# nirvanesque/headCT_foundation

Measured on AMD Instinct MI355X. Metric: CT-volumes/sec MAE pretrain step (96^3, ViT-B/16^3, mask 0.75), higher is better.
Workload: dtype bf16; 1 GPU; BASELINE config #2: MAE ViT-B/16^3, 96^3x1ch, mask 0.75, full train step (fwd+bwd+clip+AdamW+LR); per_gpu_batch=256, global_batch=256, parallelism=dp1, init=reference init, seed 42

## Files before the change

### headct_foundation_amd/_lib.py

```python
from __future__ import annotations

import ctypes as C
import os
from typing import Optional

HERE = os.path.dirname(os.path.abspath(__file__))
LIB_PATH = os.path.join(HERE, "libheadct_hip.so")

HCT_F32, HCT_BF16, HCT_F16 = 0, 1, 2
NORM_LAYERNORM, NORM_RMSNORM = 0, 1
HCT_ACT_NONE, HCT_ACT_GELU, HCT_ACT_DGELU, HCT_ACT_TANH, HCT_ACT_GELU_D, HCT_ACT_MULAUX = 0, 1, 2, 3, 4, 5
ACT_NONE, ACT_GELU, ACT_DGELU = 0, 1, 2

c_void_p, c_int, c_float, c_size_t, c_int64 = C.c_void_p, C.c_int, C.c_float, C.c_size_t, C.c_int64


class GemmArgs(C.Structure):
    _fields_ = [
        ("M", c_int), ("N", c_int), ("K", c_int),
        ("A", c_void_p), ("a_dtype", c_int), ("lda", c_int64), ("transA", c_int),
        ("B", c_void_p), ("b_dtype", c_int), ("ldb", c_int64), ("transB", c_int),
        ("C", c_void_p), ("c_dtype", c_int), ("ldc", c_int64),
        ("bias", c_void_p), ("residual", c_void_p), ("ldr", c_int64),
        ("act", c_int),
        ("aux", c_void_p), ("aux_dtype", c_int), ("ldaux", c_int64),
        ("C2", c_void_p), ("c2_dtype", c_int), ("ldc2", c_int64),
        ("alpha", c_float), ("force_generic", c_int), ("colsum_out", c_void_p), ("workspace_armed", c_int),
    ]


class GemmPlanInfo(C.Structure):
    _fields_ = [("kernel", c_int), ("epilogue_mode", c_int), ("fuse_colsum", c_int), ("row_tiles_per_wave", c_int), ("tiles", c_int),
                ("grid", c_int), ("sk_tiles", c_int), ("sk_wgs", c_int), ("splits", c_int), ("r_chunk", c_int), ("colsum_bytes", c_size_t),
                ("stream_k_offset", c_size_t), ("slab_bytes", c_size_t), ("workspace_bytes", c_size_t)]


class ProfShape(C.Structure):
    _fields_ = [("M", c_int), ("N", c_int), ("K", c_int), ("mode", c_int), ("tiles", c_int), ("sk_tiles", c_int),
                ("launches", c_int64), ("total_ms", C.c_double), ("work", C.c_double), ("bytes", C.c_double)]


def prof_shapes(lib, kernel_class: int, cap: int = 256):
    buf = (ProfShape * cap)()
    n = lib.hct_prof_shapes(kernel_class, C.cast(buf, c_void_p), cap)
    if n < 0:
        raise HctError("hct_prof_shapes failed")
    return [buf[i] for i in range(min(n, cap))]


class MaeConfig(C.Structure):
    _fields_ = [
        ("input_size", c_int), ("patch_size", c_int), ("in_chans", c_int), ("mask_ratio", C.c_double),
        ("pos_embed", c_int),
        ("encoder_depth", c_int), ("encoder_embed_dim", c_int), ("encoder_mlp_dim", c_int), ("encoder_num_heads", c_int),
        ("decoder_depth", c_int), ("decoder_embed_dim", c_int), ("decoder_mlp_dim", c_int), ("decoder_num_heads", c_int),
        ("norm_pix_loss", c_int), ("use_bias", c_int),
        ("encoder_only", c_int), ("num_register_tokens", c_int), ("final_norm_eps", c_float),
        ("lora_rank", c_int),
        ("norm_kind", c_int),
        ("dropout_rate", c_float),
    ]


class ParamInfo(C.Structure):
    _fields_ = [
        ("name", C.c_char * 96), ("ndim", c_int), ("shape", c_int64 * 5), ("offset", c_int64), ("numel", c_int64),
        ("requires_grad", c_int), ("is_matrix", c_int), ("bf16_t_offset", c_int64),
    ]


_PROTOS = {
    "hct_last_error_string": (C.c_char_p, []),
    "hct_version": (c_int, []),
    "hct_has_mfma_kernels": (c_int, []),
    "hct_gemm_workspace_bytes": (c_size_t, [C.POINTER(GemmArgs)]),
    "hct_gemm_nt_flags_offset": (c_size_t, [c_size_t]),
    "hct_gemm_describe": (c_int, [C.POINTER(GemmArgs), c_int, c_size_t, C.POINTER(GemmPlanInfo)]),
    "hct_gemm_stream_k_items": (c_int, [c_int, c_int, c_int, c_int, C.POINTER(C.c_uint32), C.POINTER(C.c_uint32)]),
    "hct_set_cu_reserve": (None, [c_int]),
    "hct_gemm": (c_int, [C.POINTER(GemmArgs), c_void_p, c_size_t, c_void_p]),
    "hct_mask_rank": (c_int, [c_void_p, c_int, c_int, c_int, c_void_p, c_void_p, c_void_p, c_void_p]),
    "hct_patch_gather": (c_int, [c_void_p, c_int, c_void_p, c_int, c_int, c_int, c_int, c_int, c_int, c_void_p, c_int, c_void_p]),
    "hct_encoder_assemble_fwd": (c_int, [c_void_p, c_int, c_void_p, c_void_p, c_void_p, c_int, c_int, c_int, c_int, c_void_p, c_void_p]),
    "hct_encoder_assemble_bwd": (c_int, [c_void_p, c_void_p, c_int, c_int, c_int, c_int, c_void_p, c_int, c_void_p, c_void_p, c_void_p, c_size_t, c_void_p]),
    "hct_assemble_bwd_workspace_bytes": (c_size_t, [c_int]),
    "hct_layernorm_fwd": (c_int, [c_void_p, c_void_p, c_void_p, c_int, c_int, c_float, c_void_p, c_int, c_void_p, c_void_p, c_void_p]),
    "hct_layernorm_bwd_workspace_bytes": (c_size_t, [c_int, c_int]),
# ... 228 lines not shown
```

### headct_foundation_amd/csrc/gemm.hip

```cpp
#include "common.h"
#include "gemm_plan.h"
#include "prof.h"

#include <cstdlib>
#include <cstring>
#include <vector>

namespace hct {

struct Epilogue {
  const float* bias;
  const float* residual;
  int64_t ldr;
  int act;
  void* aux; int aux_dtype; int64_t ldaux;
  void* C; int c_dtype; int64_t ldc;
  void* C2; int c2_dtype; int64_t ldc2;
  float alpha;
  float* colsum_partial;
  int aux_deriv;
};

__device__ __forceinline__ void store4(void* base, int dtype, int64_t off, f32x4 v) {
  if (dtype == HCT_BF16) Vec4<bf16>::store((bf16*)base + off, v);
// ... 640 lines not shown
            for (int q = 0; q < 4; ++q) {
              x0[q] *= dgelu_fast((float)t[q]);
              x1[q] *= dgelu_fast((float)t[4 + q]);
            }
          }
          if (MODE == EPI_DGELU_CS) {
            cs[h][0] += ok ? x0 : f32x4{0, 0, 0, 0};
            cs[h][1] += ok ? x1 : f32x4{0, 0, 0, 0};
          }
        }
        __builtin_amdgcn_raw_buffer_store_b128(pack(x0, x1), tb.c, vc, sc, kBf16OutPolicy);
        HCT_STORE_GUARD();
      } else {
        const f32x4 v = *reinterpret_cast<const f32x4*>(patch + pr * 256 + ((cc ^ pr) << 4));
        f32x4 x = v * e.alpha + bias[h].lo;
        if (MODE == EPI_RES_F32) x += __builtin_bit_cast(f32x4, ld[s][it]);
        __builtin_amdgcn_raw_buffer_store_b128(__builtin_bit_cast(u32x4, x), tb.c, ok ? (lane_c + h * 64) * 4u : OOB, (row0 + prow) * ldc * 4, STORE_POLICY);
        HCT_STORE_GUARD();
      }
    }
  }
}


__device__ __forceinline__ i32x4 make_srd(const void* base, uint32_t num_records) {
  const uint64_t pa = (uint64_t)base;
  return i32x4{(int)__builtin_amdgcn_readfirstlane((uint32_t)pa), (int)(__builtin_amdgcn_readfirstlane((uint32_t)(pa >> 32)) & 0xFFFF),
               (int)__builtin_amdgcn_readfirstlane(num_records), 0x00020000};
}

__device__ __forceinline__ void dma16s(i32x4 rsrc, uint32_t lds_base, uint32_t voff, uint32_t soff) {
  asm volatile("s_mov_b32 m0, %0\n\ts_nop 0\n\tbuffer_load_dwordx4 %1, %2, %3 offen lds" ::"s"(lds_base), "v"(voff), "s"(rsrc), "s"(soff)
               : "memory", "m0");
}
__device__ __forceinline__ void dma16(i32x4 rsrc, uint32_t lds_base, uint32_t voff) {
  asm volatile("s_mov_b32 m0, %0\n\ts_nop 0\n\tbuffer_load_dwordx4 %1, %2, 0 offen lds" ::"s"(lds_base), "v"(voff), "s"(rsrc) : "memory", "m0");
}

#ifdef HCT_STAMPS
__device__ uint32_t* g_stamp_ptr = nullptr;
__device__ uint32_t g_stamp_words = 0;
#define HCT_STAMP(k)                                                                                   \
  do {                                                                                                 \
    unsigned long long t_;                                                                             \
    __builtin_amdgcn_sched_barrier(0);                                                                 \
    asm volatile("s_memrealtime %0\n\ts_waitcnt lgkmcnt(0)" : "=s"(t_)::"memory");                     \
    __builtin_amdgcn_sched_barrier(0);                                                                 \
    stamps = lane == ((tile_i * 4 + (k)) & 63) ? (uint32_t)t_ : stamps;                                \
  } while (0)
#else
#define HCT_STAMP(k)
#endif

constexpr int kSkErrWord = 512;

__device__ __forceinline__ unsigned sk_pub(unsigned seq_arg) { return ((seq_arg >> 31) ? seq_arg + 1u : seq_arg) & 0x0FFFFFFFu; }

__device__ __forceinline__ uint32_t xcc_id() {
  uint32_t v;
  asm volatile("s_getreg_b32 %0, hwreg(HW_REG_XCC_ID)" : "=s"(v));
  return v & 15;
}

template <int MODE, bool SK = false, int MT = 4>
__global__ void __launch_bounds__(512, 2) gemm_bf16_nt256_kernel(int M, int N, int K, const bf16* __restrict__ A, int64_t lda,
                                                                 const bf16* __restrict__ B, int64_t ldb, Epilogue e, int ntiles, int sk_tiles, int sk_wgs, unsigned char* __restrict__ sk_ws, unsigned sk_seq) {
  __shared__ __attribute__((aligned(16))) unsigned char smem[163840];
  static_assert(MT == 4 || (MT == 3 && !SK && (MODE == EPI_PLAIN_BF16 || MODE == EPI_RES_F32)), "192-row tiles: whole tiles, plain / +residual epilogues");
  const int lane = threadIdx.x & 63, wave = __builtin_amdgcn_readfirstlane(threadIdx.x >> 6);
  const int ntn = (N + 255) >> 8;
  float* const colsum_out = e.colsum_partial;

  constexpr int NP = 2;
  uint32_t voa[NP], vob[NP];
#pragma unroll
  for (int i = 0; i < NP; ++i) {
    const int row = ((wave & 7) * NP + i) * 16 + (lane >> 2);
    const int src_chunk = (lane & 3) ^ swz64(row);
    voa[i] = (uint32_t)(row * lda * 2 + src_chunk * 16);
    vob[i] = (uint32_t)(row * ldb * 2 + src_chunk * 16);
  }
  const int wm = wave >> 1, wn = wave & 1;
  const int frow = lane & 15, fchk = lane >> 4;
  const int foff = frow * 64 + ((fchk ^ swz64(frow)) << 4);
  const int nk = K >> 5;

  i32x4 ra, rb;
  const uint32_t lds0 = (uint32_t)(size_t)((__attribute__((address_space(3))) unsigned char*)smem);
  int m0 = 0, n0 = 0;
  auto set_tile_id = [&](int id, int s0) {
    const int tm = id / ntn, tn = id - tm * ntn;
    m0 = tm * (64 * MT);
    n0 = tn << 8;
    const bf16* Ab = A + (int64_t)m0 * lda + s0 * 32;
    const bf16* Bb = B + (int64_t)n0 * ldb + s0 * 32;
    ra = make_srd(Ab, clamp_records(((int64_t)(M - m0 - 1) * lda + K - s0 * 32) * 2));
    rb = make_srd(Bb, clamp_records(((int64_t)(N - n0 - 1) * ldb + K - s0 * 32) * 2));
  };
  auto dp_id = [&](int vb) {
    const int nwg = ntiles - sk_tiles;
    const int xcd = vb & 7, q = nwg >> 3, r = nwg & 7;
    return sk_tiles + (xcd < r ? xcd * (q + 1) : r * (q + 1) + (xcd - r) * q) + (vb >> 3);
  };
  auto stage_pair = [&](int t) {
    const uint32_t b0 = lds0 + (t % 5) * 32768, b1 = lds0 + ((t + 1) % 5) * 32768;
    const uint32_t kb = (uint32_t)t * 64;
#pragma unroll
    for (int i = 0; i < NP; ++i) {
      const int c = wave * NP + i;
      if (MT == 4 || c < 4 * MT) {
        dma16s(ra, b0 + c * 1024, voa[i], kb);
        dma16s(ra, b1 + c * 1024, voa[i], kb + 64);
      }
      dma16s(rb, b0 + 16384 + c * 1024, vob[i], kb);
      dma16s(rb, b1 + 16384 + c * 1024, vob[i], kb + 64);
    }
  };
  f32x4 acc[MT][8];
  bf16x8 b_lo[4], b_hi[4], a0[MT], a1[MT];
// ... 2 lines not shown
#pragma unroll
    for (int i = 0; i < MT; ++i) af[i] = *reinterpret_cast<const bf16x8*>(sa + i * 1024);
  };
  auto rd_b = [&](int t, int half, bf16x8* bq) {
    const unsigned char* sb = smem + (t % 5) * 32768 + 16384 + wn * (128 * 64) + half * 4096 + foff;
#pragma unroll
    for (int j = 0; j < 4; ++j) bq[j] = *reinterpret_cast<const bf16x8*>(sb + j * 1024);
  };
  auto mma = [&](int half, const bf16x8* af, const bf16x8* bq) {
#pragma unroll
    for (int i = 0; i < MT; ++i)
#pragma unroll
      for (int j = 0; j < 4; ++j)
        acc[i][half * 4 + j] = __builtin_amdgcn_mfma_f32_16x16x32_bf16(bq[j], af[i], acc[i][half * 4 + j], 0, 0, 0);
  };
  auto land_all = [&]() {
    asm volatile("s_waitcnt vmcnt(0)" ::: "memory");
    __builtin_amdgcn_s_barrier();
  };
  auto land_top = [&]() {
    if (MT == 3 && wave >= 6) asm volatile("s_waitcnt vmcnt(4)" ::: "memory");
    else asm volatile("s_waitcnt vmcnt(8)" ::: "memory");
    __builtin_amdgcn_s_barrier();
  };
#ifdef HCT_STAMPS
  uint32_t stamps = 0;
  int tile_i = 0;
#endif
  const int P = nk >> 1;
  uint32_t it_first = 0, it_owner = 0;
  if (SK) stream_k_items(blockIdx.x, sk_tiles, sk_wgs, P, it_first, it_owner);
  int vb = blockIdx.x;
  uint32_t cit = 0;
  auto take_item = [&](uint32_t it) {
    set_tile_id((int)(it & 255), (int)((it >> 8) & 1023) * 2);
    cit = it;
  };
  auto next_item = [&]() -> bool {
    if (SK && it_owner) {
      take_item(it_owner);
      it_owner = 0;
      return true;
    }
    if (vb < ntiles - sk_tiles) {
      set_tile_id(dp_id(vb), 0);
      cit = (uint32_t)P << 18;
      vb += gridDim.x;
      return true;
    }
    return false;
  };
  if (SK && it_first) take_item(it_first);
  else if (!next_item()) return;
  stage_pair(0);
  while (true) {
    HCT_STAMP(0);
    const int cm0 = m0, cn0 = n0;
    const uint32_t item = cit;
    const int cns = SK ? (int)((item >> 18) & 1023) * 2 : nk;
#pragma unroll
    for (int i = 0; i < MT; ++i)
#pragma unroll
      for (int j = 0; j < 8; ++j) acc[i][j] = f32x4{0, 0, 0, 0};
    __builtin_amdgcn_s_barrier();
    stage_pair(2);
    land_top();
    HCT_STAMP(1);
    rd_a(0, a0);
    rd_b(0, 0, b_lo);
    int t = 0;
    for (; t + 5 < cns; t += 2) {
      rd_b(t, 1, b_hi);
      mma(0, a0, b_lo);
      rd_a(t + 1, a1);
      rd_b(t + 1, 0, b_lo);
      mma(1, a0, b_hi);
      rd_b(t + 1, 1, b_hi);
      mma(0, a1, b_lo);
      land_all();
      stage_pair(t + 4);
      rd_a(t + 2, a0);
      rd_b(t + 2, 0, b_lo);
      mma(1, a1, b_hi);
    }
    rd_b(t, 1, b_hi);
    mma(0, a0, b_lo);
    rd_a(t + 1, a1);
    rd_b(t + 1, 0, b_lo);
    mma(1, a0, b_hi);
    rd_b(t + 1, 1, b_hi);
    mma(0, a1, b_lo);
    land_all();
    rd_a(t + 2, a0);
    rd_b(t + 2, 0, b_lo);
    mma(1, a1, b_hi);
    rd_b(t + 2, 1, b_hi);
    mma(0, a0, b_lo);
    rd_a(t + 3, a1);
    rd_b(t + 3, 0, b_lo);
    mma(1, a0, b_hi);
    TileBias bv = {f32x4{0, 0, 0, 0}, f32x4{0, 0, 0, 0}};
    TileBias bh[2] = {bv, bv};
    if (MODE != EPI_GENERIC) tile_bias_halves<MODE>(e, cn0, wn * 128, lane, N, bh);
    rd_b(t + 3, 1, b_hi);
    mma(0, a1, b_lo);
    mma(1, a1, b_hi);
// ... 676 lines not shown
__global__ void __launch_bounds__(256) gemm_fold_kernel(const float* __restrict__ slab, int splits, int M, int N, Epilogue e) {
  const int64_t total4 = (int64_t)M * N / 4;
  for (int64_t i = (int64_t)blockIdx.x * blockDim.x + threadIdx.x; i < total4; i += (int64_t)gridDim.x * blockDim.x) {
    const int64_t idx = i * 4;
    f32x4 s = Vec4<float>::load_nt(slab + idx);
    for (int z = 1; z < splits; ++z) s += Vec4<float>::load_nt(slab + (int64_t)z * M * N + idx);
    const int m = (int)(idx / N), n = (int)(idx - (int64_t)m * N);
    epilogue4(e, m, n, s);
  }
}

static int g_cu_reserve = 0;
static GemmTuning g_tuning;

static int num_cus_total() {
  static int n = 0;
  if (n == 0) {
    int dev = 0;
    hipDeviceProp_t prop;
    if (hipGetDevice(&dev) == hipSuccess && hipGetDeviceProperties(&prop, dev) == hipSuccess) n = prop.multiProcessorCount;
    if (n <= 0) n = 256;
  }
  return n;
}

static int num_cus() { return std::max(8, num_cus_total() - g_cu_reserve); }

static Epilogue make_epilogue(const hct_gemm_args* a) {
  Epilogue e;
  e.bias = a->bias; e.residual = a->residual; e.ldr = a->ldr;
  e.aux_deriv = a->act == HCT_ACT_GELU_D || a->act == HCT_ACT_MULAUX;
  e.act = a->act == HCT_ACT_GELU_D ? HCT_ACT_GELU : a->act == HCT_ACT_MULAUX ? HCT_ACT_DGELU : a->act;
  e.aux = a->aux; e.aux_dtype = a->aux_dtype; e.ldaux = a->ldaux;
  e.C = a->C; e.c_dtype = a->c_dtype; e.ldc = a->ldc;
  e.C2 = a->C2; e.c2_dtype = a->c2_dtype; e.ldc2 = a->ldc2;
  e.alpha = a->alpha;
  e.colsum_partial = nullptr;
  return e;
}

static unsigned next_sk_seq(unsigned& seq) {
  unsigned v = (++seq) & 0x0FFFFFFFu;
  if (v == 0) v = (++seq) & 0x0FFFFFFFu;
  return g_tuning.sk_drop ? v | 0x80000000u : v;
}

static int launch_nt256(const hct_gemm_args* a, const GemmPlan& p, Epilogue e, void* workspace, hipStream_t s) {
  if (p.fuse_colsum) e.colsum_partial = (float*)workspace;
  const dim3 grid(p.grid);
  const bf16 *A = (const bf16*)a->A, *B = (const bf16*)a->B;
  if (p.row_tiles_per_wave == 3) {
    if (p.epilogue_mode == EPI_PLAIN_BF16)
      hipLaunchKernelGGL((gemm_bf16_nt256_kernel<EPI_PLAIN_BF16, false, 3>), grid, dim3(512), 0, s, a->M, a->N, a->K, A, a->lda, B, a->ldb, e,
                         p.tiles, 0, 0, (unsigned char*)nullptr, 0u);
    else
      hipLaunchKernelGGL((gemm_bf16_nt256_kernel<EPI_RES_F32, false, 3>), grid, dim3(512), 0, s, a->M, a->N, a->K, A, a->lda, B, a->ldb, e,
                         p.tiles, 0, 0, (unsigned char*)nullptr, 0u);
    HCT_CHECK_LAUNCH("hct_gemm(nt256, 192-row tiles)");
    return 0;
  }
  unsigned char* sk_ws = nullptr;
  unsigned sk_seq = 0;
  if (p.sk_tiles) {
    sk_ws = (unsigned char*)workspace + p.stream_k_offset;
    static unsigned seq = 0;
    sk_seq = next_sk_seq(seq);
    if (!a->workspace_armed)
      if (int rc = check_hip(hipMemsetAsync(sk_ws, 0, kSkHeadBytes, s), "hct_gemm(nt256): stream-K flag reset")) return rc;
  }
#define HCT_NT256(MODE_)                                                                                                             \
  do {                                                                                                                               \
    if (p.sk_tiles)                                                                                                                  \
      hipLaunchKernelGGL((gemm_bf16_nt256_kernel<MODE_, true>), grid, dim3(512), 0, s, a->M, a->N, a->K, A, a->lda, B, a->ldb, e,     \
                         p.tiles, p.sk_tiles, p.sk_wgs, sk_ws, sk_seq);                                                              \
    else                                                                                                                             \
      hipLaunchKernelGGL((gemm_bf16_nt256_kernel<MODE_, false>), grid, dim3(512), 0, s, a->M, a->N, a->K, A, a->lda, B, a->ldb, e,    \
                         p.tiles, 0, 0, (unsigned char*)nullptr, 0u);                                                                \
  } while (0)
  switch (p.epilogue_mode) {
    case EPI_PLAIN_BF16: HCT_NT256(EPI_PLAIN_BF16); break;
    case EPI_RES_F32: HCT_NT256(EPI_RES_F32); break;
    case EPI_GELU_BF16: HCT_NT256(EPI_GELU_BF16); break;
    case EPI_DGELU_BF16: if (p.fuse_colsum) HCT_NT256(EPI_DGELU_CS); else HCT_NT256(EPI_DGELU_BF16); break;
    default: HCT_NT256(EPI_GENERIC); break;
  }
#undef HCT_NT256
  HCT_CHECK_LAUNCH("hct_gemm(nt256)");
  return 0;
}

static int launch_nt128(const hct_gemm_args* a, const GemmPlan& p, const Epilogue& e, hipStream_t s) {
  hipLaunchKernelGGL(gemm_bf16_nt_kernel, dim3(p.grid), dim3(256), 0, s, a->M, a->N, a->K, (const bf16*)a->A, a->lda, (const bf16*)a->B,
                     a->ldb, e);
  HCT_CHECK_LAUNCH("hct_gemm(nt)");
  return 0;
}

static int launch_tn(const hct_gemm_args* a, const GemmPlan& p, const Epilogue& e, void* workspace, size_t workspace_bytes, hipStream_t s) {
  const bool big = p.kernel == GEMM_TN256;
  float* slab = nullptr;
  if (p.splits > 1) {
    if (workspace_bytes < p.slab_bytes || !workspace) {
      set_error("hct_gemm(%s): workspace too small (%zu < %zu)", big ? "tn256" : "tn", workspace_bytes, p.slab_bytes);
      return HCT_E_WORKSPACE;
    }
    slab = (float*)workspace;
  }
  const bf16 *A = (const bf16*)a->A, *B = (const bf16*)a->B;
  if (big)
    hipLaunchKernelGGL(gemm_bf16_tn256_kernel, dim3(p.grid), dim3(512), 0, s, a->M, a->N, a->K, p.r_chunk, A, a->lda, B, a->ldb, slab, e, p.tiles);
  else
    hipLaunchKernelGGL(gemm_bf16_tn_kernel, dim3(p.grid, p.splits), dim3(256), 0, s, a->M, a->N, a->K, p.r_chunk, A, a->lda, B, a->ldb, slab, e);
  if (slab) {
    const int64_t total4 = (int64_t)a->M * a->N / 4;
    const int blocks = (int)std::min<int64_t>(2048, (total4 + 255) / 256);
    hipLaunchKernelGGL(gemm_fold_kernel, dim3(blocks), dim3(256), 0, s, slab, p.splits, a->M, a->N, e);
  }
  HCT_CHECK_LAUNCH(big ? "hct_gemm(tn256)" : "hct_gemm(tn)");
  return 0;
}

static int launch_generic(const hct_gemm_args* a, const Epilogue& e, hipStream_t s) {
  const int64_t sam = a->transA ? 1 : a->lda, sak = a->transA ? a->lda : 1;
  const int64_t sbk = a->transB ? 1 : a->ldb, sbn = a->transB ? a->ldb : 1;
  const int vec_ok = epilogue_vec_ok(a) ? 1 : 0;
  dim3 grid((a->N + 63) / 64, (a->M + 63) / 64);
#define HCT_GEN(TA, TB)                                                                                              \
  hipLaunchKernelGGL((gemm_generic_kernel<TA, TB>), grid, dim3(256), 0, s, a->M, a->N, a->K, (const TA*)a->A, sam, sak, \
                     (const TB*)a->B, sbk, sbn, e, vec_ok)
  if (a->a_dtype == HCT_BF16 && a->b_dtype == HCT_BF16) HCT_GEN(bf16, bf16);
  else if (a->a_dtype == HCT_BF16) HCT_GEN(bf16, float);
  else if (a->b_dtype == HCT_BF16) HCT_GEN(float, bf16);
  else HCT_GEN(float, float);
#undef HCT_GEN
  HCT_CHECK_LAUNCH("hct_gemm(generic)");
  return 0;
}

static size_t tn_group_table_bytes(int n) { return align_up((size_t)n * sizeof(TnJob), 4096); }
static size_t tn_group_seg_bytes(int n) { return align_up((size_t)tn_group_seg_capacity(n) * sizeof(TnSeg), 4096); }

static int tn_group_check(const hct_gemm_args* a, int i) {
  if (!tn_group_ok(a)) {
    set_error("hct_gemm_tn_group: job %d is not a plain bf16 weight-gradient product (transA = 1, transB = 0, fp32 C, no epilogue extras, "
              "M / N multiples of 16, 16-byte aligned operands, reduction span under 4 GiB)", i);
    return HCT_E_BADARG;
  }
  return 0;
}

static int tn_group_build(const hct_gemm_args* jobs, int n, bool check, std::vector<TnJob>& tj, std::vector<TnSeg>& segs) {
  tj.resize(n);
  int tile0 = 0;
  for (int i = 0; i < n; ++i) {
    if (check)
      if (int rc = tn_group_check(jobs + i, i)) return rc;
    tj[i] = tn_group_job<bf16>(jobs + i, tile0);
    tile0 += tj[i].ntiles;
  }
  segs = tn_group_segments(tj);
  if ((int)segs.size() > tn_group_seg_capacity(n)) {
    set_error("hct_gemm_tn_group: %zu tile segments exceed the workspace's table (%d)", segs.size(), tn_group_seg_capacity(n));
    return HCT_E_WORKSPACE;
  }
  return 0;
}

}

using namespace hct;

extern "C" {

void hct_set_cu_reserve(int n) { g_cu_reserve = n < 0 ? 0 : n; }
void hct_debug_set_gemm_variant(int v) {
  if (v == -8 || v == -9) { g_tuning.sk_drop = v == -8; return; }
  if (v == -14 || v == -15) { g_tuning.mt3 = v == -14; return; }
  if (v <= -1000) { g_tuning.sk_min_k = -v - 1000; return; }
  if (v <= -100) { g_tuning.sk_gain_pairs = -v - 100; return; }
  g_tuning.nt_variant = v;
}
#ifdef HCT_STAMPS
int hct_debug_set_stamp_buffer(void* p, unsigned int n_words) {
  if (int rc = hct::check_hip(hipMemcpyToSymbol(HIP_SYMBOL(hct::g_stamp_words), &n_words, sizeof(n_words)), "stamp buffer size")) return rc;
  return hct::check_hip(hipMemcpyToSymbol(HIP_SYMBOL(hct::g_stamp_ptr), &p, sizeof(p)), "stamp buffer");
}
#endif

int hct_gemm_describe(const hct_gemm_args* a, int cus, size_t workspace_bytes, hct_gemm_plan_info* out) {
  HCT_REQUIRE(a && out && a->M >= 0 && a->N >= 0 && a->K >= 0, "hct_gemm_describe: bad arguments");
  *out = plan_gemm(a, cus > 0 ? cus : num_cus(), g_tuning, workspace_bytes);
  return 0;
}
int hct_gemm_stream_k_items(int grid, int sk_tiles, int sk_wgs, int pairs, uint32_t* first, uint32_t* owner) {
  HCT_REQUIRE(grid >= 0 && sk_tiles >= 0 && sk_wgs >= 0 && pairs > 0 && first && owner, "hct_gemm_stream_k_items: bad arguments");
  for (int wg = 0; wg < grid; ++wg) stream_k_items((unsigned)wg, sk_tiles, sk_wgs, pairs, first[wg], owner[wg]);
  return 0;
}

size_t hct_gemm_workspace_bytes(const hct_gemm_args* a) { return plan_gemm(a, num_cus(), g_tuning, kUnlimited).workspace_bytes; }
size_t hct_gemm_nt_stream_k_bytes(void) { return kSkBytes; }
size_t hct_gemm_nt_flags_offset(size_t workspace_bytes) { return ws_layout(0, workspace_bytes).stream_k_offset; }

size_t hct_gemm_tn_group_workspace_bytes(int n_jobs) { return n_jobs > 0 ? tn_group_table_bytes(n_jobs) + tn_group_seg_bytes(n_jobs) + kTnSkBytes : 0; }

int hct_gemm_tn_group_prepare(const hct_gemm_args* jobs, int n, void* workspace, size_t workspace_bytes, void* stream) {
  HCT_REQUIRE(jobs && n > 0 && n <= 4096 && workspace, "hct_gemm_tn_group_prepare: bad arguments");
  if (workspace_bytes < hct_gemm_tn_group_workspace_bytes(n) || ((uintptr_t)workspace % 256) != 0) {
    set_error("hct_gemm_tn_group: workspace too small or not 256-byte aligned (%zu < %zu)", workspace_bytes, hct_gemm_tn_group_workspace_bytes(n));
    return HCT_E_WORKSPACE;
  }
  hipStream_t s = (hipStream_t)stream;
  std::vector<TnJob> tj;
  std::vector<TnSeg> segs;
  if (int rc = tn_group_build(jobs, n, true, tj, segs)) return rc;
  for (int first = 0; first < n; first += kTnGroupChunk) {
    TnJobChunk c;
    memset(&c, 0, sizeof(c));
    const int cnt = std::min(kTnGroupChunk, n - first);
    for (int i = 0; i < cnt; ++i) c.j[i] = tj[first + i];
    hipLaunchKernelGGL(tn_group_table_kernel, dim3(1), dim3(64), 0, s, (TnJob*)workspace, c, first, cnt);
  }
  TnSeg* dsegs = (TnSeg*)((unsigned char*)workspace + tn_group_table_bytes(n));
  for (int first = 0; first < (int)segs.size(); first += kTnSegChunk) {
    TnSegChunk c;
    memset(&c, 0, sizeof(c));
    const int cnt = std::min(kTnSegChunk, (int)segs.size() - first);
    for (int i = 0; i < cnt; ++i) c.s[i] = segs[first + i];
    hipLaunchKernelGGL(tn_group_seg_kernel, dim3(1), dim3(256), 0, s, dsegs, c, first, cnt);
  }
// ... 68 lines not shown
```

### headct_foundation_amd/csrc/gemm_plan.h

```cpp
#pragma once
#include <stddef.h>
#include <stdint.h>
#include <string.h>

#include <algorithm>
#include <vector>

#include "../../include/headct_hip.h"

#ifdef __HIPCC__
#define HCT_HOST_DEVICE __host__ __device__ inline __attribute__((always_inline))
#else
#define HCT_HOST_DEVICE inline
#endif

namespace hct {

enum { EPI_GENERIC = 0, EPI_PLAIN_BF16 = 1, EPI_RES_F32 = 2, EPI_GELU_BF16 = 3, EPI_DGELU_BF16 = 4, EPI_PLAIN_F32 = 5,
       EPI_DGELU_CS = 6  };

constexpr int kSkMaxWgs = 256;
constexpr size_t kSkHeadBytes = 4096, kSkSlabBytes = 262144;
constexpr size_t kSkBytes = kSkHeadBytes + (size_t)kSkMaxWgs * kSkSlabBytes;
constexpr int kTnMaxFollowers = 1024;

struct GemmTuning {
  int nt_variant = 0;
  bool mt3 = true;
  bool sk_drop = false;
  int sk_min_k = 512;
  int sk_gain_pairs = 20;
};

enum { GEMM_GENERIC = HCT_GEMM_GENERIC, GEMM_NT128 = HCT_GEMM_NT128, GEMM_NT256 = HCT_GEMM_NT256, GEMM_TN128 = HCT_GEMM_TN128,
       GEMM_TN256 = HCT_GEMM_TN256 };
typedef hct_gemm_plan_info GemmPlan;
constexpr size_t kNoOffset = (size_t)-1;
constexpr size_t kUnlimited = (size_t)-1;

inline bool aligned_to(const void* p, size_t a) { return p == nullptr || ((uintptr_t)p % a) == 0; }
inline size_t align256(size_t v) { return (v + 255) & ~(size_t)255; }
inline int ceil_div(int v, int d) { return (v + d - 1) / d; }

inline bool epilogue_vec_ok(const hct_gemm_args* a) {
  auto ok = [](const void* p, int dt, int64_t ld) { return p == nullptr || (ld % 4 == 0 && aligned_to(p, dt == HCT_BF16 ? 8 : 16)); };
  return a->N % 4 == 0 && ok(a->C, a->c_dtype, a->ldc) && ok(a->C2, a->c2_dtype, a->ldc2) && ok(a->aux, a->aux_dtype, a->ldaux) &&
         ok(a->residual, HCT_F32, a->ldr) && aligned_to(a->bias, 16);
}

enum Path { PATH_GENERIC = 0, PATH_NT = 1, PATH_TN = 2 };

inline Path choose_path(const hct_gemm_args* a) {
  if (a->force_generic || a->a_dtype != HCT_BF16 || a->b_dtype != HCT_BF16) return PATH_GENERIC;
  if (!epilogue_vec_ok(a)) return PATH_GENERIC;
  if (!aligned_to(a->A, 16) || !aligned_to(a->B, 16) || a->lda % 8 || a->ldb % 8) return PATH_GENERIC;
  if (a->transA == 0 && a->transB == 1 && a->K % 64 == 0 && a->N % 16 == 0 && a->lda * 2 * 128 < (1ll << 31) && a->ldb * 2 * 128 < (1ll << 31))
    return PATH_NT;
  if (a->transA == 1 && a->transB == 0 && a->M % 16 == 0 && a->N % 16 == 0 && a->act == HCT_ACT_NONE && !a->bias && !a->residual &&
      (int64_t)a->K * a->lda * 2 < (1ll << 40))
    return PATH_TN;
  return PATH_GENERIC;
}

inline int epilogue_mode(const hct_gemm_args* a) {
  if (a->C2) return EPI_GENERIC;
  const bool small = a->ldc * 256 < (1ll << 28) && a->ldr * 256 < (1ll << 28) && a->ldaux * 256 < (1ll << 28);
  if (!small) return EPI_GENERIC;
  auto wide_ok = [](const void* p, int64_t ld) { return p == nullptr || (ld % 8 == 0 && aligned_to(p, 16)); };
  if (a->c_dtype == HCT_BF16 && !(a->N % 8 == 0 && wide_ok(a->C, a->ldc) && wide_ok(a->aux, a->ldaux))) return EPI_GENERIC;
  if (a->act == HCT_ACT_NONE && !a->residual && a->c_dtype == HCT_BF16) return EPI_PLAIN_BF16;
  if (a->act == HCT_ACT_NONE && a->residual && a->c_dtype == HCT_F32) return EPI_RES_F32;
  const bool is_gelu = a->act == HCT_ACT_GELU || a->act == HCT_ACT_GELU_D, is_dgelu = a->act == HCT_ACT_DGELU || a->act == HCT_ACT_MULAUX;
  if (is_gelu && !a->residual && a->c_dtype == HCT_BF16 && a->aux && a->aux_dtype == HCT_BF16) return EPI_GELU_BF16;
  if (is_dgelu && !a->residual && a->c_dtype == HCT_BF16 && a->aux_dtype == HCT_BF16) return EPI_DGELU_BF16;
  return EPI_GENERIC;
}

inline bool nt_stream_k(int K, int tiles256, int G, const GemmTuning& t, int& sk_tiles, int& sk_wgs) {
  sk_tiles = sk_wgs = 0;
  const int P = K / 64;
  if (G > kSkMaxWgs || K < t.sk_min_k || P < 8 || P > 1023) return false;
  const int rem = tiles256 % G;
  if (rem == 0 || (int64_t)(G - rem) * P < (int64_t)t.sk_gain_pairs * G) return false;
  const int gx = G / 8, nxmax = (rem + 7) / 8;
// ... 30 lines not shown
      uint32_t nf = 0;
      for (int c2 = j + 1; c2 < wx && sk_bound(c2) < tend; ++c2) ++nf;
      owner = (uint32_t)(t0 + t) | ((uint32_t)((en < tend ? en : tend) - b) << 18) | (nf << 28) | 0x80000000u;
    }
    if (!first) { first = owner; owner = 0; }
  }
}

inline bool tn256_ok(const hct_gemm_args* a, const GemmTuning& t) {
  return t.nt_variant != 128 && a->c_dtype == HCT_F32 && !a->C2 && a->ldc % 4 == 0 && a->ldc * 256 < (1ll << 28) &&
         a->lda * 2 * 64 < (1ll << 31) && a->ldb * 2 * 64 < (1ll << 31);
}

inline void tn256_split(const hct_gemm_args* a, int G, int& splits, int& r_chunk) {
  const int tiles = std::max(1, ceil_div(a->M, 256) * ceil_div(a->N, 256));
  int s = std::max(1, G / tiles);
  int per = (a->K + s - 1) / s;
  per = std::max(128, (per + 63) / 64 * 64);
  while ((int64_t)per * std::max(a->lda, a->ldb) * 2 >= (1ll << 31)) per = std::max(128, per / 2 / 64 * 64);
  r_chunk = per;
  splits = (a->K + per - 1) / per;
}

inline void tn_split(const hct_gemm_args* a, int& splits, int& r_chunk) {
  const int tiles = std::max(1, ceil_div(a->M, 128) * ceil_div(a->N, 128));
  const int steps = (a->K + 63) / 64;
  int s = (1024 + tiles - 1) / tiles;
  if (s > steps / 4) s = steps / 4;
  if (s < 1) s = 1;
  int per = (steps + s - 1) / s;
  r_chunk = per * 64;
  splits = (a->K + r_chunk - 1) / r_chunk;
}

inline int colsum_chunks(int rows, int cols) {
  const int colblk = (cols + 255) / 256;
  int chunks = (1024 + colblk - 1) / colblk;
  if (chunks > (rows + 15) / 16) chunks = (rows + 15) / 16;
  return chunks < 1 ? 1 : chunks;
}
inline size_t colsum_ws(const hct_gemm_args* a) {
  if (!a->colsum_out) return 0;
  const size_t fused = (size_t)ceil_div(a->M, 256) * 4 * a->N * sizeof(float);
  return std::max(fused, (size_t)colsum_chunks(a->M, a->N) * a->N * sizeof(float));
}

struct WsLayout { size_t head_bytes, stream_k_offset; };
inline WsLayout ws_layout(size_t colsum_bytes, size_t workspace_bytes) {
  if (workspace_bytes < align256(colsum_bytes) + kSkBytes) return WsLayout{workspace_bytes, kNoOffset};
  const size_t off = (workspace_bytes - kSkBytes) & ~(size_t)255;
  return WsLayout{off, off};
}

inline GemmPlan plan_gemm(const hct_gemm_args* a, int num_cus, const GemmTuning& t, size_t available) {
  GemmPlan p;
  memset(&p, 0, sizeof(p));
  p.row_tiles_per_wave = 4;
  p.splits = 1;
  p.stream_k_offset = kNoOffset;
  p.colsum_bytes = colsum_ws(a);
  p.workspace_bytes = p.colsum_bytes;
  const Path path = choose_path(a);
  const int G = num_cus;
  if (path == PATH_NT && a->K >= 128 && (t.nt_variant == 0 || t.nt_variant == 256)) {
    p.kernel = GEMM_NT256;
    p.epilogue_mode = epilogue_mode(a);
    p.fuse_colsum = a->colsum_out && p.epilogue_mode == EPI_DGELU_BF16;
    const int tiles256 = ceil_div(a->M, 256) * ceil_div(a->N, 256);
    p.tiles = tiles256;
    int sk_tiles = 0, sk_wgs = 0;
    if (nt_stream_k(a->K, tiles256, G, t, sk_tiles, sk_wgs)) {
      p.workspace_bytes = align256(p.colsum_bytes) + kSkBytes;
      p.stream_k_offset = ws_layout(p.colsum_bytes, available == kUnlimited ? p.workspace_bytes : available).stream_k_offset;
    }
    if (p.stream_k_offset != kNoOffset) {
      p.sk_tiles = sk_tiles;
      p.sk_wgs = sk_wgs;
      p.grid = G;
      return p;
    }
    p.grid = std::min(tiles256, G);
    if (tiles256 > G) {
      const int rounds = ceil_div(tiles256, G);
      p.grid = std::min(G, (ceil_div(tiles256, rounds) + 7) / 8 * 8);
    }
    const int tiles192 = ceil_div(a->M, 192) * ceil_div(a->N, 256);
    if (t.mt3 && (p.epilogue_mode == EPI_PLAIN_BF16 || p.epilogue_mode == EPI_RES_F32) && tiles256 < G && tiles192 <= G && tiles192 > tiles256 &&
        a->M >= 192) {
      p.row_tiles_per_wave = 3;
      p.tiles = p.grid = tiles192;
    }
    return p;
  }
  if (path == PATH_NT) {
    p.kernel = GEMM_NT128;
    p.tiles = p.grid = ceil_div(a->M, 128) * ceil_div(a->N, 128);
    return p;
  }
  if (path == PATH_TN) {
    if (tn256_ok(a, t)) {
      p.kernel = GEMM_TN256;
      tn256_split(a, G, p.splits, p.r_chunk);
      p.tiles = ceil_div(a->M, 256) * ceil_div(a->N, 256) * p.splits;
      p.grid = std::min(p.tiles, G);
    } else {
      p.kernel = GEMM_TN128;
      tn_split(a, p.splits, p.r_chunk);
      p.tiles = p.grid = ceil_div(a->M, 128) * ceil_div(a->N, 128);
    }
    p.slab_bytes = p.splits > 1 ? (size_t)p.splits * a->M * a->N * sizeof(float) : 0;
    p.workspace_bytes = p.slab_bytes;
    return p;
  }
  p.kernel = GEMM_GENERIC;
  p.tiles = p.grid = ceil_div(a->N, 64) * ceil_div(a->M, 64);
  return p;
}

inline bool tn_group_ok(const hct_gemm_args* a) {
  return a->transA == 1 && a->transB == 0 && a->a_dtype == HCT_BF16 && a->b_dtype == HCT_BF16 && a->c_dtype == HCT_F32 && !a->bias &&
         !a->residual && a->act == HCT_ACT_NONE && !a->aux && !a->C2 && !a->colsum_out && a->M > 0 && a->N > 0 && a->K > 0 && a->M % 16 == 0 &&
         a->N % 16 == 0 && a->lda % 8 == 0 && a->ldb % 8 == 0 && a->ldc % 4 == 0 && aligned_to(a->A, 16) && aligned_to(a->B, 16) &&
         aligned_to(a->C, 16) && a->A && a->B && a->C && a->ldc * 256 < (1ll << 28) && (int64_t)a->K * a->lda * 2 < 0xFFFFFFF0ll &&
         (int64_t)a->K * a->ldb * 2 < 0xFFFFFFF0ll && a->lda < (1 << 24) && a->ldb < (1 << 24);
}

template <typename BF16>
struct TnJobT {
  const BF16* A; const BF16* B; float* C;
  int M, N, R, lda, ldb, ldc;
  int tile0, ntiles, ntn, nk;
  float alpha; int pad[3];
};
struct TnSeg { int job, tile_first, count, gtile0; };
inline int tn_group_seg_capacity(int n) { return 16 * n + 64; }

template <typename BF16>
inline TnJobT<BF16> tn_group_job(const hct_gemm_args* a, int tile0) {
  TnJobT<BF16> j;
  memset(&j, 0, sizeof(j));
  j.A = (const BF16*)a->A; j.B = (const BF16*)a->B; j.C = (float*)a->C;
  j.M = a->M; j.N = a->N; j.R = a->K; j.lda = (int)a->lda; j.ldb = (int)a->ldb; j.ldc = (int)a->ldc;
  j.ntn = ceil_div(a->N, 256);
  j.ntiles = ceil_div(a->M, 256) * j.ntn;
  j.tile0 = tile0;
  j.nk = std::max(4, ((a->K + 31) / 32 + 3) / 4 * 4);
  j.alpha = a->alpha;
  return j;
}

template <typename Job>
inline std::vector<TnSeg> tn_group_segments(const std::vector<Job>& jobs) {
  std::vector<int> order(jobs.size());
  for (size_t i = 0; i < order.size(); ++i) order[i] = (int)i;
  std::stable_sort(order.begin(), order.end(), [&](int x, int y) { return jobs[x].nk > jobs[y].nk; });
  std::vector<TnSeg> segs;
  int gid = 0;
  auto emit = [&](int job, int first, int count) {
    if (!segs.empty() && segs.back().job == job && segs.back().tile_first + segs.back().count == first) segs.back().count += count;
    else segs.push_back(TnSeg{job, first, count, gid});
    gid += count;
  };
  size_t i = 0;
  while (i < order.size()) {
    size_t e = i;
    while (e < order.size() && jobs[order[e]].nk == jobs[order[i]].nk) ++e;
    struct Item { int job, first, count; };
    std::vector<Item> full, rest;
// ... 53 lines not shown
```

### include/headct_hip.h

```cpp
#ifndef HEADCT_HIP_H
#define HEADCT_HIP_H

#include <stddef.h>
#include <stdint.h>

#ifdef __cplusplus
extern "C" {
#endif

#define HCT_F32 0
#define HCT_BF16 1
#define HCT_F16 2

#define HCT_E_BADARG (-1)
#define HCT_E_UNSUPPORTED (-2)
#define HCT_E_WORKSPACE (-3)
#define HCT_E_STATE (-4)

#define HCT_ACT_NONE 0
#define HCT_ACT_GELU 1
#define HCT_ACT_DGELU 2
#define HCT_ACT_TANH 3
#define HCT_ACT_GELU_D 4
#define HCT_ACT_MULAUX 5

const char* hct_last_error_string(void);
int hct_version(void);
int hct_has_mfma_kernels(void);

typedef struct hct_gemm_args {
  int M, N, K;
  const void* A; int a_dtype; int64_t lda; int transA;
  const void* B; int b_dtype; int64_t ldb; int transB;
  void* C; int c_dtype; int64_t ldc;
  const float* bias;
  const float* residual;
  int64_t ldr;
  int act;
  void* aux; int aux_dtype; int64_t ldaux;
  void* C2; int c2_dtype; int64_t ldc2;
  float alpha;
  int force_generic;
  float* colsum_out;
  int workspace_armed;
} hct_gemm_args;

size_t hct_gemm_workspace_bytes(const hct_gemm_args* a);
size_t hct_gemm_nt_flags_offset(size_t workspace_bytes);
size_t hct_gemm_nt_stream_k_bytes(void);
void hct_set_cu_reserve(int n);
int hct_gemm(const hct_gemm_args* a, void* workspace, size_t workspace_bytes, void* stream);
#define HCT_GEMM_GENERIC 0
#define HCT_GEMM_NT128 1
#define HCT_GEMM_NT256 2
#define HCT_GEMM_TN128 3
#define HCT_GEMM_TN256 4
typedef struct hct_gemm_plan_info {
  int kernel;
  int epilogue_mode;
  int fuse_colsum;
  int row_tiles_per_wave;
  int tiles, grid;
  int sk_tiles, sk_wgs;
  int splits, r_chunk;
  size_t colsum_bytes;
  size_t stream_k_offset;
  size_t slab_bytes;
  size_t workspace_bytes;
} hct_gemm_plan_info;
int hct_gemm_describe(const hct_gemm_args* a, int num_cus, size_t workspace_bytes, hct_gemm_plan_info* out);
int hct_gemm_stream_k_items(int grid, int sk_tiles, int sk_wgs, int pairs, uint32_t* first, uint32_t* owner);
size_t hct_gemm_tn_group_workspace_bytes(int n_jobs);
int hct_gemm_tn_group_prepare(const hct_gemm_args* jobs, int n_jobs, void* workspace, size_t workspace_bytes, void* stream);
int hct_gemm_tn_group_run(const hct_gemm_args* jobs, int n_jobs, void* workspace, size_t workspace_bytes, void* stream);

int hct_mask_rank(const float* noise, int B, int L, int K, int32_t* ids_restore, int32_t* ids_shuffle,
                  float* mask, void* stream);

int hct_patch_gather(const void* x, int x_dtype , const int32_t* ids_shuffle, int B, int C, int S, int P, int L, int K,
                     void* rows, int rows_dtype, void* stream);

int hct_encoder_assemble_fwd(const void* tok, int tok_dtype, const float* cls, const float* pos,
                             const int32_t* ids_shuffle, int B, int L, int K, int D, float* h0, void* stream);
int hct_encoder_assemble_bwd(const float* dh0, const int32_t* ids_restore, int B, int L, int K, int D,
                             void* dtok, int dtok_dtype, float* dcls, float* dpos, void* workspace,
                             size_t workspace_bytes, void* stream);
size_t hct_assemble_bwd_workspace_bytes(int D);

int hct_layernorm_fwd(const float* x, const float* gamma, const float* beta, int rows, int D, float eps,
                      void* y, int y_dtype, float* mean, float* rstd, void* stream);
size_t hct_layernorm_bwd_workspace_bytes(int rows, int D);
int hct_layernorm_bwd(const void* dy, int dy_dtype, const float* x, const float* mean, const float* rstd,
                      const float* gamma, const float* dres, int rows, int D, float* dx, void* dx_shadow,
                      int shadow_dtype, float* dgamma, float* dbeta, float* dcolsum, void* workspace,
                      size_t workspace_bytes, void* stream);
int hct_layernorm_bwd_mapped(const void* dy, int dy_dtype, const float* x, const float* mean, const float* rstd,
                             const float* gamma, const float* dres, const int32_t* dres_rows, int rows, int D, float* dx,
                             void* dx_shadow, int shadow_dtype, float* dgamma, float* dbeta, float* dcolsum, void* workspace,
                             size_t workspace_bytes, void* stream);
int hct_rmsnorm_fwd(const float* x, const float* gamma, int rows, int D, float eps, void* y, int y_dtype, float* rstd,
                    void* stream);
size_t hct_rmsnorm_bwd_workspace_bytes(int rows, int D);
int hct_rmsnorm_bwd(const void* dy, int dy_dtype, const float* x, const float* rstd, const float* gamma, const float* dres,
                    int rows, int D, float* dx, void* dx_shadow, int shadow_dtype, float* dgamma, float* dcolsum,
                    void* workspace, size_t workspace_bytes, void* stream);
int hct_rmsnorm_bwd_mapped(const void* dy, int dy_dtype, const float* x, const float* rstd, const float* gamma,
                           const float* dres, const int32_t* dres_rows, int rows, int D, float* dx, void* dx_shadow,
                           int shadow_dtype, float* dgamma, float* dcolsum, void* workspace, size_t workspace_bytes,
                           void* stream);
int hct_tail_rows(const int32_t* ids_restore, int B, int L, int K, int32_t* tail_rows, int32_t* tail_inv, void* stream);
int hct_gather_rows(const void* src, const int32_t* idx, int n_rows, int row_bytes, void* dst, void* stream);

int hct_attention_fwd(const void* qkv, int B, int N, int H, int dh, int dtype, void* o, float* lse, void* stream);
int hct_attention_bwd(const void* qkv, const void* o, const void* d_o, const float* lse, int B, int N, int H,
                      int dh, int dtype, void* dqkv, void* stream);

int hct_dropout_mask(uint64_t seed, int site, int kind, int64_t n, int BH, int N, float p, unsigned char* out, void* stream);
int hct_dropout_apply(const void* x, int x_dtype, void* y, int y_dtype, const float* residual, const void* x2, void* y2,
                      int64_t batches, int64_t stride, int64_t off, int64_t seg, uint64_t seed, int site, float p, void* stream);
int hct_attention_dropout_fwd(const void* qkv, int B, int N, int H, int dh, int dtype, float p, uint64_t seed, int site, void* o,
                              float* lse, void* stream);
// ... 217 lines not shown
```

Measured before the change: 6754 CT-volumes/s.

## Stagger start of tail-round workgroups in nt256 GEMM to spread epilogue traffic

Adds a phase-offset mechanism to the persistent nt256 GEMM. Workgroups that will process one fewer tile sleep for a computed per-XCD offset before starting. The offset comes from a modeled tile time (per-K-pair cost plus fill and epilogue cost). For residual and dgelu epilogues the planner also resizes the grid to the CU count. The aim is to desynchronize epilogue and memory bursts across workgroups, at the cost of deliberate idle time and hard-coded timing constants.

Result: no change. 6767 CT-volumes/s, median of 6 (+0.2%).

```diff
diff --git a/headct_foundation_amd/_lib.py b/headct_foundation_amd/_lib.py
--- a/headct_foundation_amd/_lib.py
+++ b/headct_foundation_amd/_lib.py
@@ -32,7 +32,8 @@
 class GemmPlanInfo(C.Structure):
     _fields_ = [("kernel", c_int), ("epilogue_mode", c_int), ("fuse_colsum", c_int), ("row_tiles_per_wave", c_int), ("tiles", c_int),
                 ("grid", c_int), ("sk_tiles", c_int), ("sk_wgs", c_int), ("splits", c_int), ("r_chunk", c_int), ("colsum_bytes", c_size_t),
-                ("stream_k_offset", c_size_t), ("slab_bytes", c_size_t), ("workspace_bytes", c_size_t)]
+                ("stream_k_offset", c_size_t), ("slab_bytes", c_size_t), ("workspace_bytes", c_size_t), ("phase_slots", c_int),
+                ("phase_unit_ns", c_int), ("phase_paid_ns", c_int)]
 
 
 class ProfShape(C.Structure):
diff --git a/headct_foundation_amd/csrc/gemm.hip b/headct_foundation_amd/csrc/gemm.hip
--- a/headct_foundation_amd/csrc/gemm.hip
+++ b/headct_foundation_amd/csrc/gemm.hip
@@ -716,6 +716,11 @@
 #define HCT_STAMP(k)
 #endif
 
+__device__ __forceinline__ void phase_wait(uint32_t ns) {
+  const long long t0 = wall_clock64(), ticks = ns / 10;
+  for (int i = 0; i < 4096 && wall_clock64() - t0 < ticks; ++i) __builtin_amdgcn_s_sleep(8);
+}
+
 constexpr int kSkErrWord = 512;
 
 __device__ __forceinline__ unsigned sk_pub(unsigned seq_arg) { return ((seq_arg >> 31) ? seq_arg + 1u : seq_arg) & 0x0FFFFFFFu; }
@@ -728,7 +733,8 @@
 
 template <int MODE, bool SK = false, int MT = 4>
 __global__ void __launch_bounds__(512, 2) gemm_bf16_nt256_kernel(int M, int N, int K, const bf16* __restrict__ A, int64_t lda,
-                                                                 const bf16* __restrict__ B, int64_t ldb, Epilogue e, int ntiles, int sk_tiles, int sk_wgs, unsigned char* __restrict__ sk_ws, unsigned sk_seq) {
+                                                                 const bf16* __restrict__ B, int64_t ldb, Epilogue e, int ntiles, int sk_tiles, int sk_wgs, unsigned char* __restrict__ sk_ws, unsigned sk_seq,
+                                                                 int phase_slots, int phase_unit_ns, int phase_paid_ns) {
   __shared__ __attribute__((aligned(16))) unsigned char smem[163840];
   static_assert(MT == 4 || (MT == 3 && !SK && (MODE == EPI_PLAIN_BF16 || MODE == EPI_RES_F32)), "192-row tiles: whole tiles, plain / +residual epilogues");
   const int lane = threadIdx.x & 63, wave = __builtin_amdgcn_readfirstlane(threadIdx.x >> 6);
@@ -837,6 +843,7 @@
   };
   if (SK && it_first) take_item(it_first);
   else if (!next_item()) return;
+  if (!SK && MT == 4 && phase_slots > 0) phase_wait(phase_offset_ns_at(ntiles, (int)gridDim.x, phase_slots, phase_unit_ns, phase_paid_ns, blockIdx.x));
   stage_pair(0);
   while (true) {
     HCT_STAMP(0);
@@ -1619,10 +1626,10 @@
   if (p.row_tiles_per_wave == 3) {
     if (p.epilogue_mode == EPI_PLAIN_BF16)
       hipLaunchKernelGGL((gemm_bf16_nt256_kernel<EPI_PLAIN_BF16, false, 3>), grid, dim3(512), 0, s, a->M, a->N, a->K, A, a->lda, B, a->ldb, e,
-                         p.tiles, 0, 0, (unsigned char*)nullptr, 0u);
+                         p.tiles, 0, 0, (unsigned char*)nullptr, 0u, 0, 0, 0);
     else
       hipLaunchKernelGGL((gemm_bf16_nt256_kernel<EPI_RES_F32, false, 3>), grid, dim3(512), 0, s, a->M, a->N, a->K, A, a->lda, B, a->ldb, e,
-                         p.tiles, 0, 0, (unsigned char*)nullptr, 0u);
+                         p.tiles, 0, 0, (unsigned char*)nullptr, 0u, 0, 0, 0);
     HCT_CHECK_LAUNCH("hct_gemm(nt256, 192-row tiles)");
     return 0;
   }
@@ -1639,10 +1646,10 @@
   do {                                                                                                                               \
     if (p.sk_tiles)                                                                                                                  \
       hipLaunchKernelGGL((gemm_bf16_nt256_kernel<MODE_, true>), grid, dim3(512), 0, s, a->M, a->N, a->K, A, a->lda, B, a->ldb, e,     \
-                         p.tiles, p.sk_tiles, p.sk_wgs, sk_ws, sk_seq);                                                              \
+                         p.tiles, p.sk_tiles, p.sk_wgs, sk_ws, sk_seq, 0, 0, 0);                                                     \
     else                                                                                                                             \
       hipLaunchKernelGGL((gemm_bf16_nt256_kernel<MODE_, false>), grid, dim3(512), 0, s, a->M, a->N, a->K, A, a->lda, B, a->ldb, e,    \
-                         p.tiles, 0, 0, (unsigned char*)nullptr, 0u);                                                                \
+                         p.tiles, 0, 0, (unsigned char*)nullptr, 0u, p.phase_slots, p.phase_unit_ns, p.phase_paid_ns);               \
   } while (0)
   switch (p.epilogue_mode) {
     case EPI_PLAIN_BF16: HCT_NT256(EPI_PLAIN_BF16); break;
@@ -1743,6 +1750,16 @@
 void hct_debug_set_gemm_variant(int v) {
   if (v == -8 || v == -9) { g_tuning.sk_drop = v == -8; return; }
   if (v == -14 || v == -15) { g_tuning.mt3 = v == -14; return; }
+  if (v <= -20 && v >= -23) {
+    g_tuning.phase = v == -23 ? kPhaseAuto : -v - 20;
+    g_tuning.phase_paid_frac = 0;
+    return;
+  }
+  if (v <= -30 && v >= -38) {
+    g_tuning.phase_paid_frac = (float)(-v - 30) / 8.0f;
+    if (-v - 30 > 0 && !g_tuning.phase) g_tuning.phase = 1;
+    return;
+  }
   if (v <= -1000) { g_tuning.sk_min_k = -v - 1000; return; }
   if (v <= -100) { g_tuning.sk_gain_pairs = -v - 100; return; }
   g_tuning.nt_variant = v;
diff --git a/headct_foundation_amd/csrc/gemm_plan.h b/headct_foundation_amd/csrc/gemm_plan.h
--- a/headct_foundation_amd/csrc/gemm_plan.h
+++ b/headct_foundation_amd/csrc/gemm_plan.h
@@ -30,6 +30,9 @@
   bool sk_drop = false;
   int sk_min_k = 512;
   int sk_gain_pairs = 20;
+  int phase = -1;
+  float phase_paid_frac = 0;
+  int phase_min_rounds = 3;
 };
 
 enum { GEMM_GENERIC = HCT_GEMM_GENERIC, GEMM_NT128 = HCT_GEMM_NT128, GEMM_NT256 = HCT_GEMM_NT256, GEMM_TN128 = HCT_GEMM_TN128,
@@ -166,7 +169,7 @@
   return WsLayout{off, off};
 }
 
-inline GemmPlan plan_gemm(const hct_gemm_args* a, int num_cus, const GemmTuning& t, size_t available) {
+inline GemmPlan plan_gemm_unphased(const hct_gemm_args* a, int num_cus, const GemmTuning& t, size_t available) {
   GemmPlan p;
   memset(&p, 0, sizeof(p));
   p.row_tiles_per_wave = 4;
@@ -228,6 +231,64 @@
   }
   p.kernel = GEMM_GENERIC;
   p.tiles = p.grid = ceil_div(a->N, 64) * ceil_div(a->M, 64);
+  return p;
+}
+
+constexpr int kPhasePairNs = 1450;
+constexpr int kPhaseFillNs = 1100;
+constexpr int kPhaseEpiPlainNs = 3100 + 600;
+constexpr int kPhaseEpiResNs = 10800 + 4600;
+constexpr int kPhaseEpiGeluNs = 8200 + 2200;
+constexpr int kPhaseEpiDgeluNs = 8200 + 1000;
+constexpr int kPhaseMaxUnitNs = 250000;
+
+inline int phase_epilogue_ns(int mode) {
+  switch (mode) {
+    case EPI_PLAIN_BF16: return kPhaseEpiPlainNs;
+    case EPI_GELU_BF16: return kPhaseEpiGeluNs;
+    case EPI_DGELU_BF16: case EPI_DGELU_CS: return kPhaseEpiDgeluNs;
+    default: return kPhaseEpiResNs;
+  }
+}
+constexpr int kPhaseAuto = -1;
+inline int phase_default(int mode) { return mode == EPI_RES_F32 || mode == EPI_DGELU_BF16 || mode == EPI_DGELU_CS ? 2 : 0; }
+inline int64_t phase_tile_ns(int K, int mode) { return (int64_t)kPhasePairNs * (K / 64) + kPhaseFillNs + phase_epilogue_ns(mode); }
+
+HCT_HOST_DEVICE uint32_t phase_offset_ns_at(int tiles, int grid, int slots, int unit_ns, int paid_ns, unsigned w) {
+  if (slots <= 0 || grid <= 0 || w >= (unsigned)grid) return 0;
+  const int rem = tiles % grid;
+  if (rem == 0 || (int)w < rem) {
+    if (paid_ns <= 0) return 0;
+    const int per_xcd = ((rem ? rem : grid) + 7) >> 3;
+    return (uint32_t)((int64_t)(w >> 3) * paid_ns / per_xcd);
+  }
+  return (uint32_t)((int64_t)((w - (unsigned)rem) >> 3) * unit_ns / slots);
+}
+inline uint32_t phase_offset_ns(const GemmPlan& p, unsigned w) {
+  return phase_offset_ns_at(p.tiles, p.grid, p.phase_slots, p.phase_unit_ns, p.phase_paid_ns, w);
+}
+
+inline void plan_phase(GemmPlan& p, int K, int G, const GemmTuning& t) {
+  if (p.kernel != GEMM_NT256 || p.sk_tiles || p.row_tiles_per_wave != 4 || p.tiles <= G) return;
+  const int mode = p.fuse_colsum ? EPI_DGELU_CS : p.epilogue_mode;
+  const int phase = t.phase == kPhaseAuto ? phase_default(mode) : t.phase;
+  if (!phase) return;
+  const int grid = phase == 2 ? G : p.grid;
+  const int64_t unit = phase_tile_ns(K, mode);
+  if (unit > kPhaseMaxUnitNs) return;
+  const int rem = p.tiles % grid, rounds = ceil_div(p.tiles, grid);
+  const float frac = std::min(1.0f, std::max(0.0f, t.phase_paid_frac));
+  const int paid = rounds >= t.phase_min_rounds ? (int)(frac * (float)unit) : 0;
+  if (rem == 0 && paid == 0) return;
+  p.grid = grid;
+  p.phase_slots = rem ? ceil_div(grid - rem, 8) : ceil_div(grid, 8);
+  p.phase_unit_ns = (int)unit;
+  p.phase_paid_ns = paid;
+}
+
+inline GemmPlan plan_gemm(const hct_gemm_args* a, int num_cus, const GemmTuning& t, size_t available) {
+  GemmPlan p = plan_gemm_unphased(a, num_cus, t, available);
+  plan_phase(p, a->K, num_cus, t);
   return p;
 }
 
diff --git a/include/headct_hip.h b/include/headct_hip.h
--- a/include/headct_hip.h
+++ b/include/headct_hip.h
@@ -67,6 +67,9 @@
   size_t stream_k_offset;
   size_t slab_bytes;
   size_t workspace_bytes;
+  int phase_slots;
+  int phase_unit_ns;
+  int phase_paid_ns;
 } hct_gemm_plan_info;
 int hct_gemm_describe(const hct_gemm_args* a, int num_cus, size_t workspace_bytes, hct_gemm_plan_info* out);
 int hct_gemm_stream_k_items(int grid, int sk_tiles, int sk_wgs, int pairs, uint32_t* first, uint32_t* owner);
```
